# nv-tlabs/LION

Hardware: NVIDIA H100
Metric: shapes/sec (1000-step DDPM, 2048 latent pts, B=32) (higher is better)
Workload: dtype tf32 (fp32 storage/accumulate)

## Files before the change

include/lion_b200.h:

```cpp
#ifndef LION_B200_H
#define LION_B200_H
#include <stddef.h>
#ifdef __cplusplus
extern "C" {
#endif

typedef struct LionCtx LionCtx;
typedef struct LionModel LionModel;

int lion_version(void);
const char* lion_last_error(void);
int lion_ctx_create(int device, LionCtx** out);
int lion_ctx_destroy(LionCtx* ctx);
int lion_ctx_last_launches(LionCtx* ctx);
int lion_ctx_last_conv_group(LionCtx* ctx);
int lion_ctx_last_conv_stage_taps(LionCtx* ctx);
int lion_ctx_set_conv_whole_slabs(LionCtx* ctx, int on);
unsigned lion_ctx_generation(LionCtx* ctx);
int lion_ctx_timeline(LionCtx* ctx, unsigned long long* t_ns, char* names, int max_entries);
size_t lion_ctx_arena_bytes(LionCtx* ctx);
size_t lion_workspace_bytes(LionCtx* ctx);

int lion_avg_voxelize(const float* features, const int* coords, float* out, int* ind, int* cnt,
                      int B, int C, int N, int r, void* stream);
int lion_trilinear_devoxelize(const float* grid, const float* coords, float* out, int* inds, float* wgts,
                              int B, int C, int N, int r, int is_training, void* stream);
int lion_furthest_point_sampling(const float* coords, int* idx, int B, int N, int M, void* stream);
int lion_gather(const float* features, const int* idx, float* out, int B, int C, int N, int M, void* stream);
int lion_ball_query(const float* centers, const float* points, int* out, int B, int N, int M, float radius, int K,
                    void* stream);
int lion_grouping(const float* features, const int* idx, float* out, int B, int C, int N, int M, int U, void* stream);
int lion_three_nn_interpolate(const float* points, const float* centers, const float* centers_features, float* out,
                              int* idx, float* wgt, int B, int C, int N, int M, void* stream);
int lion_voxel_coords(const float* coords, float* norm_coords, int* vox, int B, int N, int r, int normalize, float eps,
                      void* stream);

int lion_avg_voxelize_backward(const float* grad_y , const int* ind , const int* cnt ,
                               float* grad_x , int B, int C, int N, int r, void* stream);
int lion_trilinear_devoxelize_backward(const float* grad_y , const int* inds , const float* wgts ,
                                       float* grad_x , int B, int C, int N, int r, void* stream);
// ... 16 lines not shown
                      int B, int N, void* stream);
#define LION_FWD_CONV_FP16 1
int lion_unet_forward_flags(LionModel* m, const float* x, const float* t, const float* style, const float* clip, float* out,
                            int B, int N, int flags, void* stream);
int lion_unet_cache_style(LionModel* m, const float* style, const float* clip, int B, void* stream);
int lion_style_encoder_forward(LionModel* m, const float* x, float* out, int B, int N, void* stream);
int lion_pvconv_fwd(LionModel* m, const float* features, const float* coords, const float* style, float* out,
                    int B, int N, void* stream);
int lion_sa_module_fwd(LionModel* m, const float* features, const float* coords, const float* style,
                       float* out_features, float* out_coords, int B, int N, void* stream);
int lion_fp_module_fwd(LionModel* m, const float* points_coords, const float* centers_coords,
                       const float* centers_features, const float* points_features, const float* style, float* out,
                       int B, int N, int M, void* stream);
int lion_linear_attention_fwd(LionModel* m, const float* x, float* out, int B, int N, void* stream);
int lion_shared_mlp_fwd(LionModel* m, const float* x, const float* style, float* out, int B, int R, void* stream);
int lion_adagn_fwd(LionModel* m, const float* x, const float* style, float* out, int B, int R, void* stream);
int lion_se3d_fwd(LionCtx* ctx, const float* w1, const float* w2, const float* x, float* out, int B, int C, int V, void* stream);
int lion_swish_fwd(const float* x, float* out, size_t n, void* stream);
int lion_conv3d_gn_fwd(LionModel* m, const float* x, float* out, double* gn_sum, double* gn_sqsum, int B, void* stream);
int lion_conv3d_gn_fwd_flags(LionModel* m, const float* x, float* out, double* gn_sum, double* gn_sqsum, int B, int flags,
                             void* stream);
int lion_pvconv_conv1_probe(LionModel* m, const float* features, const float* coords, int path, float* out,
                            double* gn_sum, double* gn_sqsum, int* path_taken, int B, int N, void* stream);
int lion_sa_mlp_probe(LionModel* m, const float* features, const float* coords, const float* style, int path,
                      float* centers, double* gn_sum, double* gn_sqsum, float* scale, float* shift, float* pool_mm,
                      int* path_taken, int B, int N, void* stream);
int lion_pvconv_probe(LionModel* m, const float* features, const float* coords, const float* style, float* raw1, float* act1,
                      float* raw2, float* rawp, double* sums, float* affine, float* fused, float* out, int* conv2_kernel,
                      int B, int N, void* stream);
int lion_pvconv_probe_flags(LionModel* m, const float* features, const float* coords, const float* style, float* raw1,
                            float* act1, float* raw2, float* rawp, double* sums, float* affine, float* fused, float* out,
                            int* conv2_kernel, int B, int N, int flags, void* stream);
int lion_attention_probe(LionModel* m, const float* x, float* qkv, float* o, float* out, int B, int N, void* stream);
int lion_fp_probe(LionModel* m, const float* points_coords, const float* centers_coords, const float* centers_features,
                  const float* points_features, const float* style, int* nn_idx, float* nn_wgt, float* cat, float* raw,
                  float* act, double* gn_sum, double* gn_sqsum, float* scale, float* shift, int B, int N, int M, void* stream);
int lion_unet_probe(LionModel* m, const float* x, const float* t, const float* style, const float* clip, float* out,
                    void* const* taps, int ntaps, int* style_table, int n_style, int B, int N, void* stream);
int lion_global_prior_forward(LionModel* m, const float* x, const float* t, const float* clip, float* out, int B,
                              void* stream);
int lion_global_prior_probe(LionModel* m, const float* x, const float* t, const float* clip, float* out,
                            void* const* taps, int ntaps, int B, void* stream);
int lion_global_prior_step(LionModel* m, const float* x, const float* t, const float* clip, float* out, int B,
                           void* stream);
size_t lion_global_prior_saved_floats(LionModel* m, int B);
int lion_global_prior_forward_train(LionModel* m, const float* x, const float* t, const float* clip,
// ... 74 lines not shown
```

lion_b200/_lib.py:

```python
import ctypes as C
import os
import threading

import torch

_HERE = os.path.dirname(os.path.abspath(__file__))
LIB_PATH = os.path.join(_HERE, "csrc", "liblion_b200.so")


class LionError(RuntimeError):
    pass


_lib = None
_lock = threading.Lock()
c_f = C.c_void_p


def _proto(lib):
    i, f, d, sz, vp = C.c_int, C.c_float, C.c_double, C.c_size_t, C.c_void_p
    P = lambda *a: list(a)
    sig = {
        "lion_version": ([], i),
        "lion_last_error": ([], C.c_char_p),
        "lion_ctx_create": (P(i, C.POINTER(vp)), i),
        "lion_ctx_destroy": (P(vp), i),
        "lion_ctx_last_launches": (P(vp), i),
        "lion_ctx_last_conv_group": (P(vp), i),
        "lion_ctx_last_conv_stage_taps": (P(vp), i),
        "lion_ctx_set_conv_whole_slabs": (P(vp, i), i),
        "lion_ctx_arena_bytes": (P(vp), sz),
        "lion_ctx_generation": (P(vp), C.c_uint),
        "lion_ctx_timeline": (P(vp, vp, vp, i), i),
        "lion_avg_voxelize": (P(vp, vp, vp, vp, vp, i, i, i, i, vp), i),
        "lion_trilinear_devoxelize": (P(vp, vp, vp, vp, vp, i, i, i, i, i, vp), i),
        "lion_furthest_point_sampling": (P(vp, vp, i, i, i, vp), i),
        "lion_gather": (P(vp, vp, vp, i, i, i, i, vp), i),
        "lion_ball_query": (P(vp, vp, vp, i, i, i, f, i, vp), i),
        "lion_grouping": (P(vp, vp, vp, i, i, i, i, i, vp), i),
        "lion_three_nn_interpolate": (P(vp, vp, vp, vp, vp, vp, i, i, i, i, vp), i),
        "lion_voxel_coords": (P(vp, vp, vp, i, i, i, i, f, vp), i),
        "lion_avg_voxelize_backward": (P(vp, vp, vp, vp, i, i, i, i, vp), i),
        "lion_trilinear_devoxelize_backward": (P(vp, vp, vp, vp, i, i, i, i, vp), i),
        "lion_grouping_backward": (P(vp, vp, vp, i, i, i, i, i, vp), i),
        "lion_three_nn_interpolate_backward": (P(vp, vp, vp, vp, i, i, i, i, vp), i),
        "lion_gather_backward": (P(vp, vp, vp, i, i, i, i, vp), i),
        "lion_model_create": (P(vp, i, C.POINTER(i), i, C.POINTER(vp), i, C.POINTER(vp)), i),
        "lion_model_destroy": (P(vp), i),
        "lion_model_refresh": (P(vp), i),
        "lion_unet_forward": (P(vp, vp, vp, vp, vp, vp, i, i, vp), i),
        "lion_unet_forward_flags": (P(vp, vp, vp, vp, vp, vp, i, i, i, vp), i),
        "lion_unet_cache_style": (P(vp, vp, vp, i, vp), i),
        "lion_style_encoder_forward": (P(vp, vp, vp, i, i, vp), i),
        "lion_pvconv_fwd": (P(vp, vp, vp, vp, vp, i, i, vp), i),
        "lion_sa_module_fwd": (P(vp, vp, vp, vp, vp, vp, i, i, vp), i),
        "lion_fp_module_fwd": (P(vp, vp, vp, vp, vp, vp, vp, i, i, i, vp), i),
        "lion_linear_attention_fwd": (P(vp, vp, vp, i, i, vp), i),
        "lion_shared_mlp_fwd": (P(vp, vp, vp, vp, i, i, vp), i),
        "lion_global_prior_forward": (P(vp, vp, vp, vp, vp, i, vp), i),
        "lion_adagn_fwd": (P(vp, vp, vp, vp, i, i, vp), i),
        "lion_se3d_fwd": (P(vp, vp, vp, vp, vp, i, i, i, vp), i),
        "lion_swish_fwd": (P(vp, vp, sz, vp), i),
        "lion_ddpm_update": (P(vp, vp, vp, vp, vp, vp, f, sz, vp, i, vp), i),
        "lion_ddpm_set_step": (P(vp, vp, i, i, vp), i),
        "lion_ddpm_next_step": (P(vp, vp, i, vp), i),
        "lion_ddpm_fetch_noise": (P(vp, vp, vp, sz, vp), i),
        "lion_conv3d_gn_fwd": (P(vp, vp, vp, vp, vp, i, vp), i),
        "lion_conv3d_gn_fwd_flags": (P(vp, vp, vp, vp, vp, i, i, vp), i),
        "lion_pvconv_conv1_probe": (P(vp, vp, vp, i, vp, vp, vp, C.POINTER(i), i, i, vp), i),
        "lion_sa_mlp_probe": (P(vp, vp, vp, vp, i, vp, vp, vp, vp, vp, vp, C.POINTER(i), i, i, vp), i),
        "lion_pvconv_probe": (P(vp, vp, vp, vp, vp, vp, vp, vp, vp, vp, vp, vp, C.POINTER(i), i, i, vp), i),
        "lion_pvconv_probe_flags": (P(vp, vp, vp, vp, vp, vp, vp, vp, vp, vp, vp, vp, C.POINTER(i), i, i, i, vp), i),
        "lion_attention_probe": (P(vp, vp, vp, vp, vp, i, i, vp), i),
        "lion_fp_probe": (P(vp, vp, vp, vp, vp, vp, vp, vp, vp, vp, vp, vp, vp, vp, vp, i, i, i, vp), i),
        "lion_unet_probe": (P(vp, vp, vp, vp, vp, vp, C.POINTER(vp), i, C.POINTER(i), i, i, i, vp), i),
        "lion_global_prior_step": (P(vp, vp, vp, vp, vp, i, vp), i),
        "lion_global_prior_probe": (P(vp, vp, vp, vp, vp, C.POINTER(vp), i, i, vp), i),
        "lion_global_prior_saved_floats": (P(vp, i), sz),
        "lion_global_prior_forward_train": (P(vp, vp, vp, vp, vp, vp, vp, i, vp), i),
        "lion_global_prior_backward": (P(vp, vp, vp, vp, vp, vp, C.POINTER(vp), i, i, vp), i),
        "lion_global_prior_backward_probe": (P(vp, vp, vp, vp, vp, vp, C.POINTER(vp), i, C.POINTER(vp), i, i, vp), i),
        "lion_workspace_bytes": (P(vp), sz),
        "lion_ddim_update": (P(vp, vp, vp, vp, vp, vp, sz, vp, vp), i),
        "lion_ddim_set_step": (P(vp, vp, vp, i, i, i, vp), i),
        "lion_ddim_next_step": (P(vp, vp, vp, i, i, vp), i),
        "lion_scheduler_step": (P(vp, vp, vp, vp, vp, vp, sz, vp), i),
        "lion_ode_state_bytes": ([], sz),
        "lion_ode_init": (P(vp, vp, vp, sz, d, d, d, d, i, vp), i),
        "lion_ode_stage": (P(vp, vp, vp, vp, sz, i, vp, vp, i, vp), i),
        "lion_ode_rhs": (P(vp, vp, vp, vp, sz, i, d, d, d, vp, vp), i),
        "lion_ode_norms": (P(vp, vp, vp, vp, sz, i, vp, vp), i),
        "lion_ode_control": (P(vp, vp, sz, i, vp), i),
# ... 192 lines not shown
```

lion_b200/csrc/common.cuh:

```cuda
#pragma once
#include <cuda_runtime.h>
#include <cstdint>
#include <cstdio>
#include <cstdarg>
#include <cstring>
#include <string>
#include <vector>
#include <mutex>

namespace lion {

enum : int { LION_OK = 0, LION_ERR_CUDA = -1, LION_ERR_ARG = -2, LION_ERR_OOM = -3, LION_ERR_STATE = -4 };

void set_error(const char* fmt, ...);
const char* get_error();

#define LION_CHECK_CUDA(expr)                                                          \
  do {                                                                                 \
    cudaError_t _e = (expr);                                                           \
    if (_e != cudaSuccess) {                                                           \
      lion::set_error("%s:%d: %s -> %s", __FILE__, __LINE__, #expr, cudaGetErrorString(_e)); \
      return lion::LION_ERR_CUDA;                                                      \
    }                                                                                  \
  } while (0)
// ... 13 lines not shown
  } while (0)

constexpr int LION_MAX_STAMPS = 256;
struct Ctx {
  int device = 0;
  int num_sms = 132;
  int l2_bytes = 50 << 20;
  cudaStream_t stream = nullptr;
  cudaStream_t aux = nullptr;
  char* base = nullptr;
  char* zgrid = nullptr;
  size_t zgrid_cap = 0, zgrid_need = 0;
  size_t cap = 0;
  size_t off = 0;
  size_t peak = 0;
  unsigned generation = 0;
  std::mutex* mu = nullptr;
  bool dry = false;
  int launches = 0;
  int conv_smem_cap = 0;
  int conv_group_blocks = 0;
  int conv_stage_taps = 0;
  bool conv_whole_slabs = false;
  unsigned long long* d_stamps = nullptr;
  int n_stamps = 0;
  char stamp_names[LION_MAX_STAMPS][24];

  void reset() { off = 0; peak = 0; launches = 0; zgrid_need = 0; n_stamps = 0; }
  void* alloc(size_t bytes) {
    size_t a = (off + 255) & ~size_t(255);
    off = a + bytes;
    if (off > peak) peak = off;
    if (dry) return (void*)(uintptr_t)(0x1000 + a);
    return base + a;
  }
  template <typename T> T* alloc_n(size_t n) { return (T*)alloc(n * sizeof(T)); }
  size_t mark() const { return off; }
  void release(size_t m) { off = m; }
};

int ctx_reserve(Ctx* c, size_t bytes);

#define LION_LAUNCH_ON(ctx, stream, kernel, grid, block, smem, ...)                    \
  do {                                                                                 \
    if (!(ctx)->dry) {                                                                 \
      kernel<<<(grid), (block), (smem), (stream)>>>(__VA_ARGS__);                      \
// ... 92 lines not shown
```

lion_b200/csrc/net.cu:

```cuda
#include <algorithm>
#include <deque>
#include <memory>
#include <cstdlib>
#include <cmath>
#include "common.cuh"
#include "packed_kernels.cuh"
#include "model.cuh"
#include "../../include/lion_b200.h"

namespace lion {

static thread_local char g_err[1024] = "";
void set_error(const char* fmt, ...) {
  va_list ap;
  va_start(ap, fmt);
  vsnprintf(g_err, sizeof(g_err), fmt, ap);
  va_end(ap);
}
const char* get_error() { return g_err; }

int ctx_reserve(Ctx* c, size_t bytes) {
  if (bytes <= c->cap) return 0;
  cudaStreamCaptureStatus st = cudaStreamCaptureStatusNone;
  cudaStreamIsCapturing(c->stream, &st);
// ... 454 lines not shown
  if (N > VOXP_MAXN || r > 32) { set_error("voxelisation: N=%d (max %d) or r=%d (max 32) unsupported", N, VOXP_MAXN, r); return LION_ERR_ARG; }
  v.nc = f.c->alloc_n<float4>((size_t)f.B * N);
  v.order = f.c->alloc_n<int>((size_t)f.B * N);
  v.ppos = f.c->alloc_n<int>((size_t)f.B * N);
  v.len = f.c->alloc_n<int>((size_t)f.B * N);
  int P = (r + 2) * (r + 2) * (r + 2);
  v.occ_stride = (P + 63) / 64 + 4;
  v.occ = f.c->alloc_n<unsigned char>((size_t)f.B * v.occ_stride);
  LION_TRY(memset_async(f.c, v.occ, 0, (size_t)f.B * v.occ_stride, s));
  if (sparse_conv1_wanted(N, r)) {
    v.cidx = f.c->alloc_n<int>((size_t)f.B * N);
    v.nocc = f.c->alloc_n<int>((size_t)f.B);
    v.vgrid = f.c->alloc_n<int>((size_t)f.B * P);
    LION_TRY(memset_async(f.c, v.vgrid, 0xff, (size_t)f.B * P * sizeof(int), s));
  }
  LION_LAUNCH_ON(f.c, s, k_vox_prep, f.B, VOXP_THREADS, 0, c4, v.nc, v.order, v.ppos, v.len, v.occ, v.occ_stride, N, r, v.cidx, v.nocc,
                 v.vgrid);
  LION_TRY(check_launch(f.c, "vox_prep"));
  f.vox.push_back(v);
  *out = &f.vox.back();
  return 0;
}

struct Conv1Out { float4* raw = nullptr; double* ssum = nullptr; double* ssq = nullptr; float4* g_in = nullptr; bool sparse = false; };
template <typename F>
static int pvconv_conv1(Fwd& f, const PVConvBlk& p, PF feat, const VoxPrep* vp, int path, Conv1Out& o, F&& after_scatter) {
  const int N = feat.R, r = p.r, rp = r + 2, P = rp * rp * rp, Gin = p.cin / 4, Gout = p.cout / 4;
  ConvGeom geo1 = geom_grid(r);
  geo1.occ = vp->occ; geo1.occ_stride = vp->occ_stride;
  const bool sparse_ok = vp->cidx && ygemm_usable(p.c1y) && feat.G == p.c1y.cin_pad / 4;
  if (path == 2 && !sparse_ok) { set_error("PVConv: the sparse first convolution cannot serve this layer / grid"); return LION_ERR_ARG; }
  if (path == 1 && !conv_tc_usable(p.c1, geo1)) { set_error("PVConv: no tensor-core packing of the first convolution"); return LION_ERR_ARG; }
  const bool sparse1 = path == 0 ? sparse_ok : path == 2;
  o.sparse = sparse1;
  PF xc;
  if (sparse1) {
    xc = alloc_pf(f, Gin, N);
    LION_LAUNCH(f.c, k_scatter_compact, dim3(cdiv(N, 128), Gin, f.B), 128, 0, feat.p, vp->order, vp->cidx, vp->len, vp->nocc, xc.p, Gin, N);
  } else {
    size_t zbytes = sizeof(float4) * ((size_t)f.B * Gin * P + 2 * ((size_t)rp * rp + rp + 8));
    if (zbytes > f.c->zgrid_need) f.c->zgrid_need = zbytes;
    o.g_in = f.c->dry ? (float4*)(uintptr_t)0x1000 : (float4*)f.c->zgrid + ((size_t)rp * rp + rp + 8);
    LION_LAUNCH(f.c, k_scatter, dim3(cdiv(N, 128), Gin, f.B), 128, 0, feat.p, vp->order, vp->ppos, vp->len, o.g_in, Gin, N, P);
  }
  stamp(f.c, f.c->stream, " scatter");
  LION_TRY(after_scatter());
  float4* raw1 = alloc_vg(f, Gout, r);
  o.raw = raw1;
  LION_TRY(poison_vg(f, raw1, Gout, r));
  if (sparse1) {
    const int ld = 27 * p.c1.cout_pad;
    float* y = f.c->alloc_n<float>((size_t)f.B * N * ld);
    LION_TRY(ygemm_run(f.c, p.c1y, xc.p, y, ld, vp->nocc, f.B, N));
    double *s1, *q1;
    LION_TRY(alloc_stats(f, p.c1.cout_pad, &s1, &q1));
    const int nwarp = 4;
    const size_t smem = (size_t)nwarp * (32 * (p.c1.cout_pad + 2) * sizeof(float) + SPG_LIST * sizeof(unsigned));
    static DevOnce attr_once;
    if (attr_once.need()) {
      LION_CHECK_CUDA(cudaFuncSetAttribute(k_sparse_conv_gather<32>, cudaFuncAttributeMaxDynamicSharedMemorySize, 96 * 1024));
      LION_CHECK_CUDA(cudaFuncSetAttribute(k_sparse_conv_gather<64>, cudaFuncAttributeMaxDynamicSharedMemorySize, 96 * 1024));
      LION_CHECK_CUDA(cudaFuncSetAttribute(k_sparse_conv_gather<32>, cudaFuncAttributePreferredSharedMemoryCarveout, cudaSharedmemCarveoutMaxShared));
      LION_CHECK_CUDA(cudaFuncSetAttribute(k_sparse_conv_gather<64>, cudaFuncAttributePreferredSharedMemoryCarveout, cudaSharedmemCarveoutMaxShared));
      LION_CHECK_CUDA(cudaFuncSetAttribute(k_act_grid<false>, cudaFuncAttributePreferredSharedMemoryCarveout, cudaSharedmemCarveoutMaxShared));
      LION_CHECK_CUDA(cudaFuncSetAttribute(k_act_grid<true>, cudaFuncAttributePreferredSharedMemoryCarveout, cudaSharedmemCarveoutMaxShared));
      LION_CHECK_CUDA(cudaFuncSetAttribute(k_scatter_compact, cudaFuncAttributePreferredSharedMemoryCarveout, cudaSharedmemCarveoutMaxShared));
    }
    const dim3 grid(cdiv(r * r * r, 32 * nwarp), f.B);
    if (p.c1.cout_pad == 32)
      LION_LAUNCH(f.c, k_sparse_conv_gather<32>, grid, 32 * nwarp, smem, y, ld, vp->vgrid, p.c1.bias, raw1, s1, q1, p.c1.cout_pad, r, N);
    else
      LION_LAUNCH(f.c, k_sparse_conv_gather<64>, grid, 32 * nwarp, smem, y, ld, vp->vgrid, p.c1.bias, raw1, s1, q1, p.c1.cout_pad, r, N);
    LION_TRY(check_launch(f.c, "sparse conv1"));
    o.ssum = s1; o.ssq = q1;
  } else {
    LION_TRY(alloc_stats(f, p.c1.cout_pad, &o.ssum, &o.ssq));
    LION_TRY(run_conv(f, p.c1, o.g_in, Gin, raw1, Gout, o.ssum, o.ssq, geo1));
  }
  return 0;
}

static int pvconv_fwd(Fwd& f, const PVConvBlk& p, PF feat, const float4* c4, float4* dst, int Gd, int g_off) {
  int N = feat.R, r = p.r, rp = r + 2, P = rp * rp * rp, Gin = p.cin / 4, Gout = p.cout / 4;
  if (feat.G != Gin) { set_error("PVConv: got %d input channels, expected %d", feat.G * 4, p.cin); return LION_ERR_ARG; }
  VoxPrep* vp;
  LION_TRY(get_vox(f, f.c->stream, c4, N, r, &vp));
  size_t mk = f.c->mark();
  ConvGeom geo = geom_grid(r);
  const ConvW& pw = p.point.conv[0];
  PF rawp;
  AffSrc ap;
  PrepJob jp, j1;
  Conv1Out c1;
  LION_TRY(pvconv_conv1(f, p, feat, vp, 0, c1, [&]() -> int {
    rawp = alloc_pf(f, Gout, N);
    return conv_gn_deferred(f, pw, feat.p, feat.G, rawp.p, Gout, geom_rows(N), p.point.gn[0], (double)N, ap, jp);
  }));
  const bool sparse1 = c1.sparse;
  float4 *raw1 = c1.raw, *g_in = c1.g_in;
  AffSrc a1;
  const double V = (double)r * r * r;
  j1 = prep_job(f, p.g1, c1.ssum, c1.ssq, p.c1.cout_pad, V, nullptr, nullptr, a1);
  LION_TRY(run_prep(f, j1, &jp));
  stamp(f.c, f.c->stream, " conv1");
  const bool h2 = f.conv_f16 && p.c2.tc16.w;
  const int Gact = h2 ? Gout / 2 : Gout;
  float4* act1 = alloc_vg(f, Gact, r);
  LION_TRY(poison_vg(f, act1, Gact, r));
  {
    const int nb_act = cdiv(P, 256 * ACT_U);
    const dim3 grid(nb_act + (sparse1 ? 0 : cdiv(N, 256)), Gact, f.B);
    if (h2)
      LION_LAUNCH(f.c, k_act_grid<true>, grid, 256, 0, raw1, act1, a1, Gout, p.cout, rp, P, nb_act, vp->ppos, g_in, Gin, N);
    else
      LION_LAUNCH(f.c, k_act_grid<false>, grid, 256, 0, raw1, act1, a1, Gout, p.cout, rp, P, nb_act, vp->ppos, g_in, Gin, N);
  }
  stamp(f.c, f.c->stream, " act1");
  float4* raw2 = alloc_vg(f, Gout, r);
  LION_TRY(poison_vg(f, raw2, Gout, r));
  AffSrc a2;
  LION_TRY(conv_gn(f, p.c2, act1, Gact, raw2, Gout, geo, p.g2, V, p.se1, p.se2, a2, h2));
  stamp(f.c, f.c->stream, " conv2");
  if (f.pv) {
    PvRecord& R = *f.pv;
    R.raw1 = raw1; R.act1 = act1; R.raw2 = raw2; R.rawp = rawp.p; R.act1_f16 = h2;
    R.a1 = a1; R.ap = ap; R.a2 = a2;
    R.conv2 = !conv_tc_usable(p.c2, geo) ? 0 : f.c->conv_group_blocks ? f.c->conv_group_blocks : 1;
  }
  if (p.has_attn) {
    PF fused = alloc_pf(f, Gout, N);
    LION_LAUNCH(f.c, k_devox_fuse, dim3(cdiv(N, 128), Gout, f.B), 128, 0, raw2, vp->nc, a2.scale, a2.shift, rawp.p, ap,
                fused.p, Gout, p.cout, N, r, P, Gout, 0);
    LION_TRY(check_launch(f.c, "pvconv"));
    if (f.pv) f.pv->fused = fused.p;
    if (Gd != Gout || g_off != 0) {
      PF t = alloc_pf(f, Gout, N);
      LION_TRY(attn_fwd(f, p.attn, fused, t.p, Gout, 0));
      LION_LAUNCH(f.c, k_copy_groups, dim3(cdiv(N, 256), Gout, f.B), 256, 0, t.p, dst, Gout, Gd, g_off, N);
// ... 533 lines not shown
    delete h;
    return LION_ERR_STATE;
  }
  *out = h;
  return 0;
}
extern "C" int lion_ctx_destroy(LionCtx* h) {
  if (!h) return 0;
  if (h->c.base) cudaFree(h->c.base);
  if (h->c.zgrid) cudaFree(h->c.zgrid);
  if (h->c.aux) cudaStreamDestroy(h->c.aux);
  if (h->c.d_stamps) cudaFree(h->c.d_stamps);
  delete h;
  return 0;
}
extern "C" int lion_ctx_last_launches(LionCtx* h) { return h ? h->c.launches : 0; }
extern "C" int lion_ctx_last_conv_group(LionCtx* h) { return h ? h->c.conv_group_blocks : 0; }
extern "C" int lion_ctx_last_conv_stage_taps(LionCtx* h) { return h ? h->c.conv_stage_taps : 0; }
extern "C" int lion_ctx_set_conv_whole_slabs(LionCtx* h, int on) {
  LION_REQUIRE(h, "lion_ctx_set_conv_whole_slabs: null context");
  h->c.conv_whole_slabs = on != 0;
  return 0;
}
extern "C" unsigned lion_ctx_generation(LionCtx* h) { return h ? h->c.generation : 0; }
extern "C" int lion_ctx_timeline(LionCtx* h, unsigned long long* t_ns, char* names, int max_entries) {
  LION_REQUIRE(h && t_ns && names && max_entries >= 0, "lion_ctx_timeline: null argument");
  if (!h->c.d_stamps) { set_error("lion_ctx_timeline: the context was created without LION_TIMELINE=1"); return LION_ERR_STATE; }
  int n = h->c.n_stamps < max_entries ? h->c.n_stamps : max_entries;
  LION_CHECK_CUDA(cudaSetDevice(h->c.device));
  LION_CHECK_CUDA(cudaDeviceSynchronize());
  LION_CHECK_CUDA(cudaMemcpy(t_ns, h->c.d_stamps, (size_t)n * sizeof(unsigned long long), cudaMemcpyDeviceToHost));
  for (int i = 0; i < n; ++i) memcpy(names + (size_t)i * 24, h->c.stamp_names[i], 24);
  return n;
}
extern "C" size_t lion_ctx_arena_bytes(LionCtx* h) { return h ? h->c.cap : 0; }
extern "C" size_t lion_workspace_bytes(LionCtx* h) { return h ? h->c.cap + h->c.zgrid_cap : 0; }

extern "C" int lion_model_create(LionCtx* ctx, int kind, const int* desc, int ndesc, const float* const* params,
                                 int nparams, LionModel** out) {
  LION_REQUIRE(ctx && out && (desc || ndesc == 0) && (params || nparams == 0), "lion_model_create: null argument");
  LION_CHECK_CUDA(cudaSetDevice(ctx->c.device));
  std::unique_ptr<LionModel> h(new LionModel());
  Model* m = &h->m;
  m->ctx = &ctx->c; m->kind = kind;
  m->desc.assign(desc, desc + ndesc);
  m->params.assign(params, params + nparams);
// ... 295 lines not shown
      LION_CHECK_CUDA(cudaMemcpy2DAsync(gn_sum, sizeof(double) * cout, ssum, sizeof(double) * w.cout_pad, sizeof(double) * cout, B,
                                        cudaMemcpyDeviceToDevice, f.c->stream));
      LION_CHECK_CUDA(cudaMemcpy2DAsync(gn_sqsum, sizeof(double) * cout, ssq, sizeof(double) * w.cout_pad, sizeof(double) * cout, B,
                                        cudaMemcpyDeviceToDevice, f.c->stream));
    }
    return check_launch(f.c, "lion_conv3d_gn_fwd");
  });
}

extern "C" int lion_pvconv_conv1_probe(LionModel* h, const float* features, const float* coords, int path, float* out,
                                       double* gn_sum, double* gn_sqsum, int* path_taken, int B, int N, void* stream) {
  LION_REQUIRE(h && h->m.kind == LION_KIND_PVCONV, "lion_pvconv_conv1_probe: not a pvconv model");
  LION_REQUIRE(features && coords && out && gn_sum && gn_sqsum && path >= 0 && path <= 2 && B > 0 && N > 0,
               "lion_pvconv_conv1_probe: bad arguments");
  Model* m = &h->m;
  return two_pass(m, stream, B, [&](Fwd& f) -> int {
    const PVConvBlk& p = m->block->pv;
    const int r = p.r, rp = r + 2, P = rp * rp * rp, Gout = p.cout / 4;
    PF x = to_pf(f, features, m->desc[0], N);
    float4* c4 = to_c4(f, coords, N);
    VoxPrep* vp;
    LION_TRY(get_vox(f, f.c->stream, c4, N, r, &vp));
    Conv1Out c1;
    LION_TRY(pvconv_conv1(f, p, x, vp, path, c1, [] { return 0; }));
    if (!c1.sparse)
      LION_LAUNCH(f.c, k_act_grid<false>, dim3(cdiv(N, 256), Gout, B), 256, 0, c1.raw, nullptr, AffSrc{}, Gout, p.cout, rp, P, 0,
                  vp->ppos, c1.g_in, p.cin / 4, N);
    LION_LAUNCH(f.c, k_vg_to_cm, dim3(cdiv(r * r * r, 256), Gout, B), 256, 0, c1.raw, out, p.cout, Gout, r);
    if (!f.c->dry) {
      LION_CHECK_CUDA(cudaMemcpy2DAsync(gn_sum, sizeof(double) * p.cout, c1.ssum, sizeof(double) * p.c1.cout_pad,
                                        sizeof(double) * p.cout, B, cudaMemcpyDeviceToDevice, f.c->stream));
      LION_CHECK_CUDA(cudaMemcpy2DAsync(gn_sqsum, sizeof(double) * p.cout, c1.ssq, sizeof(double) * p.c1.cout_pad,
                                        sizeof(double) * p.cout, B, cudaMemcpyDeviceToDevice, f.c->stream));
      if (path_taken) *path_taken = c1.sparse ? 2 : 1;
    }
    return check_launch(f.c, "lion_pvconv_conv1_probe");
  });
}

extern "C" int lion_sa_mlp_probe(LionModel* h, const float* features, const float* coords, const float* style, int path,
                                 float* centers, double* gn_sum, double* gn_sqsum, float* scale, float* shift, float* pool_mm,
                                 int* path_taken, int B, int N, void* stream) {
  LION_REQUIRE(h && h->m.kind == LION_KIND_SA, "lion_sa_mlp_probe: not an SA model");
  LION_REQUIRE(features && coords && (style || h->m.desc[4] == 0) && centers && gn_sum && gn_sqsum && scale && shift && pool_mm &&
               path >= 0 && path <= 2 && B > 0 && N > 0, "lion_sa_mlp_probe: bad arguments");
  Model* m = &h->m;
  const SABlk& s = m->block->sa;
  LION_REQUIRE((int)s.mlp.conv.size() <= MLP_REC_MAX, "lion_sa_mlp_probe: more than %d layers", MLP_REC_MAX);
  LION_REQUIRE(path != 2 || sa_fused_usable(s), "lion_sa_mlp_probe: the fused kernels do not serve this module");
  return two_pass(m, stream, B, [&](Fwd& f) -> int {
    MlpRecord rec;
    rec.force = path;
    f.rec = &rec;
    LION_TRY(style_affine_all(f, style ? style : f.c->alloc_n<float>((size_t)B * 4)));
    PF x = to_pf(f, features, s.cfeat, N);
    Level lv{to_c4(f, coords, N), N};
    lv.centers = f.c->alloc_n<float4>((size_t)B * s.m);
    PF o = alloc_pf(f, s.mlp.cout() / 4, s.m);
    LION_TRY(sa_geometry(f, f.c->stream, s, lv, 0));
// ... 314 lines not shown
```

lion_b200/csrc/packed_kernels.cuh:

```cuda
#pragma once
#include <cuda_fp16.h>
#include "common.cuh"
#include "point_core.cuh"
#include "model.cuh"

namespace lion {

__device__ __forceinline__ float4 f4_max(float4 a, float4 b) {
  return make_float4(fmaxf(a.x, b.x), fmaxf(a.y, b.y), fmaxf(a.z, b.z), fmaxf(a.w, b.w));
}
__device__ __forceinline__ float4 f4_scale(float4 a, float s) { return make_float4(a.x * s, a.y * s, a.z * s, a.w * s); }
__device__ __forceinline__ float4 f4_add(float4 a, float4 b) { return make_float4(a.x + b.x, a.y + b.y, a.z + b.z, a.w + b.w); }
__device__ __forceinline__ float4 f4_fma(float4 a, float s, float4 c) {
  return make_float4(fmaf(a.x, s, c.x), fmaf(a.y, s, c.y), fmaf(a.z, s, c.z), fmaf(a.w, s, c.w));
}

__global__ void k_make_coords(const float4* __restrict__ x, float4* __restrict__ c4, int total) {
  int i = blockIdx.x * blockDim.x + threadIdx.x;
  if (i >= total) return;
  float4 v = x[i];
  v.w = 0.0f;
  c4[i] = v;
}

// ... 122 lines not shown
        const unsigned e = list[i0 + k];
        const float* src = yb + (size_t)(e >> 10) * ldy + ((e >> 5) & 31) * C + lane * CPL;
        if (CPL == 2) val[k] = __ldg(reinterpret_cast<const float2*>(src));
        else val[k] = make_float2(__ldg(src), 0.0f);
        jj[k] = (int)(e & 31);
      }
    }
#pragma unroll
    for (int k = 0; k < SPG_BATCH; ++k) {
      if (jj[k] >= 0) {
        float* a = acc + jj[k] * PITCH + lane * CPL;
        a[0] += val[k].x;
        if (CPL == 2) a[1] += val[k].y;
      }
    }
  }
  __syncwarp();
}

template <int C>
__global__ void __launch_bounds__(128)
k_sparse_conv_gather(const float* __restrict__ y, int ldy, const int* __restrict__ vgrid, const float* __restrict__ bias,
                     float4* __restrict__ out, double* __restrict__ ssum, double* __restrict__ ssq, int stat_stride,
                     int r, int Nrows) {
  static_assert(C == 32 || C == 64, "two (or one) channels per lane");
  constexpr int CPL = C / 32;
  constexpr int PITCH = C + 2;
  extern __shared__ float s_acc[];
  __shared__ float s_red[2][4][C];
  const int b = blockIdx.y, lane = threadIdx.x & 31, wid = threadIdx.x >> 5, nw = blockDim.x >> 5;
  const int rp = r + 2, P = rp * rp * rp, V = r * r * r;
  const int q = (blockIdx.x * nw + wid) * 32 + lane;
  const bool live = q < V;
  int p = 0;
  if (live) { int z = q % r, yy = (q / r) % r, x = q / (r * r); p = ((x + 1) * rp + (yy + 1)) * rp + (z + 1); }
  float* acc = s_acc + (size_t)wid * 32 * PITCH;
  const int* vg = vgrid + (size_t)b * P;
  int nb[27];
#pragma unroll
  for (int t = 0; t < 27; ++t) {
    const int off = ((t / 9) - 1) * rp * rp + (((t / 3) % 3) - 1) * rp + ((t % 3) - 1);
    nb[t] = live ? __ldg(vg + p + off) : -1;
  }
  {
    float bv[CPL];
#pragma unroll
    for (int k = 0; k < CPL; ++k) bv[k] = bias ? bias[lane * CPL + k] : 0.0f;
    for (int j = 0; j < 32; ++j)
#pragma unroll
      for (int k = 0; k < CPL; ++k) acc[j * PITCH + lane * CPL + k] = bv[k];
  }
  const float* yb = y + (size_t)b * Nrows * ldy;
  unsigned* list = reinterpret_cast<unsigned*>(s_acc + (size_t)nw * 32 * PITCH) + wid * SPG_LIST;
  int n = 0;
#pragma unroll
  for (int t = 0; t < 27; ++t) {
    const int v = nb[t];
    const unsigned m = __ballot_sync(0xffffffffu, v >= 0);
    if (n + 32 > SPG_LIST) { spg_flush<C>(acc, list, n, yb, ldy, lane); n = 0; }
    if (v >= 0) list[n + __popc(m & ((1u << lane) - 1u))] = ((unsigned)v << 10) | ((unsigned)t << 5) | (unsigned)lane;
    n += __popc(m);
  }
  spg_flush<C>(acc, list, n, yb, ldy, lane);
  if (live) {
#pragma unroll
    for (int g = 0; g < C / 4; ++g) {
      const float* a = acc + lane * PITCH + g * 4;
      out[((size_t)b * (C / 4) + g) * P + p] = make_float4(a[0], a[1], a[2], a[3]);
    }
  }
  float cs[2][CPL], cq[2][CPL];
#pragma unroll
  for (int k = 0; k < CPL; ++k) { cs[0][k] = cs[1][k] = 0.0f; cq[0][k] = cq[1][k] = 0.0f; }
  const int nlive = max(0, min(32, V - ((int)blockIdx.x * nw + wid) * 32));
  for (int j = 0; j < nlive; j += 2) {
#pragma unroll
    for (int h = 0; h < 2; ++h) {
      if (j + h < nlive) {
#pragma unroll
        for (int k = 0; k < CPL; ++k) { const float a = acc[(j + h) * PITCH + lane * CPL + k]; cs[h][k] += a; cq[h][k] = fmaf(a, a, cq[h][k]); }
      }
    }
  }
#pragma unroll
  for (int k = 0; k < CPL; ++k) { s_red[0][wid][lane * CPL + k] = cs[0][k] + cs[1][k]; s_red[1][wid][lane * CPL + k] = cq[0][k] + cq[1][k]; }
  __syncthreads();
  if (threadIdx.x < C) {
    float a = 0.0f, qq = 0.0f;
    for (int w = 0; w < nw; ++w) { a += s_red[0][w][threadIdx.x]; qq += s_red[1][w][threadIdx.x]; }
    atomicAdd(ssum + (size_t)b * stat_stride + threadIdx.x, (double)a);
    atomicAdd(ssq + (size_t)b * stat_stride + threadIdx.x, (double)qq);
  }
}

__global__ void k_scatter(const float4* __restrict__ feat, const int* __restrict__ s_order, const int* __restrict__ s_ppos,
                          const int* __restrict__ s_len, float4* __restrict__ grid, int G, int N, int P) {
  int b = blockIdx.z, g = blockIdx.y;
// ... 249 lines not shown
    double var = gq / n - mean * mean;
    if (var < 0) var = 0;
    const float rstd = (float)(1.0 / sqrt(var + 1e-5));
    const float f = a.fb[(size_t)b * a.fb_stride + c], bb = a.fb[(size_t)b * a.fb_stride + C + c];
    const float ga = a.gamma[c], be = a.beta[c];
    s_aff[threadIdx.x] = rstd * ga * f;
    s_aff[4 + threadIdx.x] = (be - (float)mean * rstd * ga) * f + bb;
  }
  __syncthreads();
  s = make_float4(s_aff[0], s_aff[1], s_aff[2], s_aff[3]);
  t = make_float4(s_aff[4], s_aff[5], s_aff[6], s_aff[7]);
}

constexpr int ACT_U = 4;
__device__ __forceinline__ float4 h8_pack(float4 a, float4 b) {
  union { __half2 h[4]; float4 f; } u;
  u.h[0] = __floats2half2_rn(a.x, a.y); u.h[1] = __floats2half2_rn(a.z, a.w);
  u.h[2] = __floats2half2_rn(b.x, b.y); u.h[3] = __floats2half2_rn(b.z, b.w);
  return u.f;
}

template <bool F16>
__global__ void k_act_grid(const float4* __restrict__ in, float4* __restrict__ out, AffSrc aff, int G, int C, int rp, int P,
                           int nb_act, const int* __restrict__ us_ppos, float4* __restrict__ us_grid, int us_G, int us_N) {
  constexpr int NG = F16 ? 2 : 1;
  int b = blockIdx.z, g = blockIdx.y;
  if ((int)blockIdx.x >= nb_act) {
    int sidx = ((int)blockIdx.x - nb_act) * blockDim.x + threadIdx.x;
    if (sidx >= us_N) return;
    int pp = us_ppos[(size_t)b * us_N + sidx];
    if (pp >= 0)
      for (int gg = g; gg < us_G; gg += gridDim.y) us_grid[((size_t)b * us_G + gg) * P + pp] = make_float4(0.f, 0.f, 0.f, 0.f);
    return;
  }
  float4 s[NG], t[NG];
#pragma unroll
  for (int k = 0; k < NG; ++k) {
    if (k) __syncthreads();
    aff_block_load(aff, b, NG * g + k, C, s[k], t[k]);
  }
  const float4* src = in + ((size_t)b * G + NG * g) * P;
  float4* dst = out + ((size_t)b * (G / NG) + g) * P;
  const int p0 = blockIdx.x * (blockDim.x * ACT_U) + threadIdx.x;
  float4 v[ACT_U][NG];
  bool interior[ACT_U];
  const unsigned rp_m = 0xffffffffu / (unsigned)rp + 1u;
#pragma unroll
  for (int u = 0; u < ACT_U; ++u) {
    int p = p0 + u * blockDim.x;
    const int q = (int)__umulhi((unsigned)p, rp_m), x = (int)__umulhi((unsigned)q, rp_m);
    const int z = p - q * rp, y = q - x * rp;
    interior[u] = p < P && z >= 1 && z <= rp - 2 && y >= 1 && y <= rp - 2 && x >= 1 && x <= rp - 2;
#pragma unroll
    for (int k = 0; k < NG; ++k) {
      v[u][k] = make_float4(0.f, 0.f, 0.f, 0.f);
      if (interior[u]) v[u][k] = __ldcs(src + (size_t)k * P + p);
    }
  }
#pragma unroll
  for (int u = 0; u < ACT_U; ++u) {
    int p = p0 + u * blockDim.x;
    if (p < P) {
      float4 r = make_float4(0.f, 0.f, 0.f, 0.f);
      if (interior[u]) {
        if constexpr (F16) r = h8_pack(f4_swish(f4_affine(v[u][0], s[0], t[0])), f4_swish(f4_affine(v[u][1], s[1], t[1])));
        else r = f4_tf32(f4_swish(f4_affine(v[u][0], s[0], t[0])));
      }
      dst[p] = r;
    }
  }
}

template <int POOL>
__global__ void k_act_rows(const float4* __restrict__ in, float4* __restrict__ out, AffSrc aff, int G, int C, int R_out, int Gd,
                           int g_off, int flags) {
  int b = blockIdx.z, g = blockIdx.y;
  int i = blockIdx.x * blockDim.x + threadIdx.x;
  float4 s, t;
  aff_block_load(aff, b, g, C, s, t);
  if (i >= R_out) return;
  const float4* src = in + ((size_t)b * G + g) * (size_t)R_out * POOL + (size_t)i * POOL;
  float4 r = f4_affine(src[0], s, t);
  if (!(flags & 2)) r = f4_swish(r);
#pragma unroll 4
  for (int k = 1; k < POOL; ++k) r = f4_max(r, f4_swish(f4_affine(src[k], s, t)));
  if (flags & 1) r = f4_tf32(r);
  out[((size_t)b * Gd + g_off + g) * R_out + i] = r;
}

__global__ void k_act_rows_pool32(const float4* __restrict__ in, float4* __restrict__ out, AffSrc aff, int G, int C, int R_out,
                                  int Gd, int g_off) {
// ... 404 lines not shown
```

Before: 3.052.

## Skip raw stores for empty voxel warps in sparse conv1 using occupancy mask

The sparse conv1 gather kernel now writes a per-warp bitmask of output voxels that have at least one occupied neighbour. It skips storing raw outputs for voxels with none, unless whole-output storage is requested. The activation kernel reads this mask and substitutes a precomputed constant, the swish of the affine-transformed bias, for inactive interior voxels instead of loading raw values. This is meant to cut global memory traffic for the sparse voxel grid, at the cost of an extra mask buffer, per-element mask lookups, and a debug flag plus probe to force dense behaviour.

```diff
diff --git a/include/lion_b200.h b/include/lion_b200.h
--- a/include/lion_b200.h
+++ b/include/lion_b200.h
@@ -16,6 +16,7 @@
 int lion_ctx_last_conv_group(LionCtx* ctx);
 int lion_ctx_last_conv_stage_taps(LionCtx* ctx);
 int lion_ctx_set_conv_whole_slabs(LionCtx* ctx, int on);
+int lion_ctx_set_sparse_conv1_dense(LionCtx* ctx, int on);
 unsigned lion_ctx_generation(LionCtx* ctx);
 int lion_ctx_timeline(LionCtx* ctx, unsigned long long* t_ns, char* names, int max_entries);
 size_t lion_ctx_arena_bytes(LionCtx* ctx);
@@ -78,6 +79,8 @@
                              void* stream);
 int lion_pvconv_conv1_probe(LionModel* m, const float* features, const float* coords, int path, float* out,
                             double* gn_sum, double* gn_sqsum, int* path_taken, int B, int N, void* stream);
+int lion_pvconv_conv1_mask_probe(LionModel* m, const float* features, const float* coords, int* vgrid, unsigned* mask, int B,
+                                 int N, void* stream);
 int lion_sa_mlp_probe(LionModel* m, const float* features, const float* coords, const float* style, int path,
                       float* centers, double* gn_sum, double* gn_sqsum, float* scale, float* shift, float* pool_mm,
                       int* path_taken, int B, int N, void* stream);
diff --git a/lion_b200/_lib.py b/lion_b200/_lib.py
--- a/lion_b200/_lib.py
+++ b/lion_b200/_lib.py
@@ -29,6 +29,7 @@
         "lion_ctx_last_conv_group": (P(vp), i),
         "lion_ctx_last_conv_stage_taps": (P(vp), i),
         "lion_ctx_set_conv_whole_slabs": (P(vp, i), i),
+        "lion_ctx_set_sparse_conv1_dense": (P(vp, i), i),
         "lion_ctx_arena_bytes": (P(vp), sz),
         "lion_ctx_generation": (P(vp), C.c_uint),
         "lion_ctx_timeline": (P(vp, vp, vp, i), i),
@@ -68,6 +69,7 @@
         "lion_conv3d_gn_fwd": (P(vp, vp, vp, vp, vp, i, vp), i),
         "lion_conv3d_gn_fwd_flags": (P(vp, vp, vp, vp, vp, i, i, vp), i),
         "lion_pvconv_conv1_probe": (P(vp, vp, vp, i, vp, vp, vp, C.POINTER(i), i, i, vp), i),
+        "lion_pvconv_conv1_mask_probe": (P(vp, vp, vp, vp, vp, i, i, vp), i),
         "lion_sa_mlp_probe": (P(vp, vp, vp, vp, i, vp, vp, vp, vp, vp, vp, C.POINTER(i), i, i, vp), i),
         "lion_pvconv_probe": (P(vp, vp, vp, vp, vp, vp, vp, vp, vp, vp, vp, vp, C.POINTER(i), i, i, vp), i),
         "lion_pvconv_probe_flags": (P(vp, vp, vp, vp, vp, vp, vp, vp, vp, vp, vp, vp, C.POINTER(i), i, i, i, vp), i),
diff --git a/lion_b200/csrc/common.cuh b/lion_b200/csrc/common.cuh
--- a/lion_b200/csrc/common.cuh
+++ b/lion_b200/csrc/common.cuh
@@ -59,6 +59,7 @@
   int conv_group_blocks = 0;
   int conv_stage_taps = 0;
   bool conv_whole_slabs = false;
+  bool sparse_conv1_dense = false;
   unsigned long long* d_stamps = nullptr;
   int n_stamps = 0;
   char stamp_names[LION_MAX_STAMPS][24];
diff --git a/lion_b200/csrc/net.cu b/lion_b200/csrc/net.cu
--- a/lion_b200/csrc/net.cu
+++ b/lion_b200/csrc/net.cu
@@ -500,9 +500,11 @@
   return 0;
 }
 
-struct Conv1Out { float4* raw = nullptr; double* ssum = nullptr; double* ssq = nullptr; float4* g_in = nullptr; bool sparse = false; };
+struct Conv1Out { float4* raw = nullptr; double* ssum = nullptr; double* ssq = nullptr; float4* g_in = nullptr; bool sparse = false;
+                  const unsigned* mask = nullptr; };
 template <typename F>
-static int pvconv_conv1(Fwd& f, const PVConvBlk& p, PF feat, const VoxPrep* vp, int path, Conv1Out& o, F&& after_scatter) {
+static int pvconv_conv1(Fwd& f, const PVConvBlk& p, PF feat, const VoxPrep* vp, int path, bool whole_raw, Conv1Out& o,
+                        F&& after_scatter) {
   const int N = feat.R, r = p.r, rp = r + 2, P = rp * rp * rp, Gin = p.cin / 4, Gout = p.cout / 4;
   ConvGeom geo1 = geom_grid(r);
   geo1.occ = vp->occ; geo1.occ_stride = vp->occ_stride;
@@ -545,12 +547,17 @@
       LION_CHECK_CUDA(cudaFuncSetAttribute(k_scatter_compact, cudaFuncAttributePreferredSharedMemoryCarveout, cudaSharedmemCarveoutMaxShared));
     }
     const dim3 grid(cdiv(r * r * r, 32 * nwarp), f.B);
+    unsigned* mask = f.c->alloc_n<unsigned>((size_t)f.B * cdiv(r * r * r, 32));
+    const bool whole = whole_raw || f.c->sparse_conv1_dense;
     if (p.c1.cout_pad == 32)
-      LION_LAUNCH(f.c, k_sparse_conv_gather<32>, grid, 32 * nwarp, smem, y, ld, vp->vgrid, p.c1.bias, raw1, s1, q1, p.c1.cout_pad, r, N);
+      LION_LAUNCH(f.c, k_sparse_conv_gather<32>, grid, 32 * nwarp, smem, y, ld, vp->vgrid, p.c1.bias, raw1, s1, q1, p.c1.cout_pad, r, N,
+                  mask, whole);
     else
-      LION_LAUNCH(f.c, k_sparse_conv_gather<64>, grid, 32 * nwarp, smem, y, ld, vp->vgrid, p.c1.bias, raw1, s1, q1, p.c1.cout_pad, r, N);
+      LION_LAUNCH(f.c, k_sparse_conv_gather<64>, grid, 32 * nwarp, smem, y, ld, vp->vgrid, p.c1.bias, raw1, s1, q1, p.c1.cout_pad, r, N,
+                  mask, whole);
     LION_TRY(check_launch(f.c, "sparse conv1"));
     o.ssum = s1; o.ssq = q1;
+    o.mask = mask;
   } else {
     LION_TRY(alloc_stats(f, p.c1.cout_pad, &o.ssum, &o.ssq));
     LION_TRY(run_conv(f, p.c1, o.g_in, Gin, raw1, Gout, o.ssum, o.ssq, geo1));
@@ -570,12 +577,13 @@
   AffSrc ap;
   PrepJob jp, j1;
   Conv1Out c1;
-  LION_TRY(pvconv_conv1(f, p, feat, vp, 0, c1, [&]() -> int {
+  LION_TRY(pvconv_conv1(f, p, feat, vp, 0, f.pv != nullptr, c1, [&]() -> int {
     rawp = alloc_pf(f, Gout, N);
     return conv_gn_deferred(f, pw, feat.p, feat.G, rawp.p, Gout, geom_rows(N), p.point.gn[0], (double)N, ap, jp);
   }));
   const bool sparse1 = c1.sparse;
   float4 *raw1 = c1.raw, *g_in = c1.g_in;
+  const unsigned* mask1 = f.c->sparse_conv1_dense ? nullptr : c1.mask;
   AffSrc a1;
   const double V = (double)r * r * r;
   j1 = prep_job(f, p.g1, c1.ssum, c1.ssq, p.c1.cout_pad, V, nullptr, nullptr, a1);
@@ -589,9 +597,11 @@
     const int nb_act = cdiv(P, 256 * ACT_U);
     const dim3 grid(nb_act + (sparse1 ? 0 : cdiv(N, 256)), Gact, f.B);
     if (h2)
-      LION_LAUNCH(f.c, k_act_grid<true>, grid, 256, 0, raw1, act1, a1, Gout, p.cout, rp, P, nb_act, vp->ppos, g_in, Gin, N);
+      LION_LAUNCH(f.c, k_act_grid<true>, grid, 256, 0, raw1, act1, a1, Gout, p.cout, rp, P, nb_act, vp->ppos, g_in, Gin, N, mask1,
+                  p.c1.bias);
     else
-      LION_LAUNCH(f.c, k_act_grid<false>, grid, 256, 0, raw1, act1, a1, Gout, p.cout, rp, P, nb_act, vp->ppos, g_in, Gin, N);
+      LION_LAUNCH(f.c, k_act_grid<false>, grid, 256, 0, raw1, act1, a1, Gout, p.cout, rp, P, nb_act, vp->ppos, g_in, Gin, N, mask1,
+                  p.c1.bias);
   }
   stamp(f.c, f.c->stream, " act1");
   float4* raw2 = alloc_vg(f, Gout, r);
@@ -1171,6 +1181,11 @@
   h->c.conv_whole_slabs = on != 0;
   return 0;
 }
+extern "C" int lion_ctx_set_sparse_conv1_dense(LionCtx* h, int on) {
+  LION_REQUIRE(h, "lion_ctx_set_sparse_conv1_dense: null context");
+  h->c.sparse_conv1_dense = on != 0;
+  return 0;
+}
 extern "C" unsigned lion_ctx_generation(LionCtx* h) { return h ? h->c.generation : 0; }
 extern "C" int lion_ctx_timeline(LionCtx* h, unsigned long long* t_ns, char* names, int max_entries) {
   LION_REQUIRE(h && t_ns && names && max_entries >= 0, "lion_ctx_timeline: null argument");
@@ -1512,10 +1527,10 @@
     VoxPrep* vp;
     LION_TRY(get_vox(f, f.c->stream, c4, N, r, &vp));
     Conv1Out c1;
-    LION_TRY(pvconv_conv1(f, p, x, vp, path, c1, [] { return 0; }));
+    LION_TRY(pvconv_conv1(f, p, x, vp, path, true, c1, [] { return 0; }));
     if (!c1.sparse)
       LION_LAUNCH(f.c, k_act_grid<false>, dim3(cdiv(N, 256), Gout, B), 256, 0, c1.raw, nullptr, AffSrc{}, Gout, p.cout, rp, P, 0,
-                  vp->ppos, c1.g_in, p.cin / 4, N);
+                  vp->ppos, c1.g_in, p.cin / 4, N, nullptr, nullptr);
     LION_LAUNCH(f.c, k_vg_to_cm, dim3(cdiv(r * r * r, 256), Gout, B), 256, 0, c1.raw, out, p.cout, Gout, r);
     if (!f.c->dry) {
       LION_CHECK_CUDA(cudaMemcpy2DAsync(gn_sum, sizeof(double) * p.cout, c1.ssum, sizeof(double) * p.c1.cout_pad,
@@ -1525,6 +1540,26 @@
       if (path_taken) *path_taken = c1.sparse ? 2 : 1;
     }
     return check_launch(f.c, "lion_pvconv_conv1_probe");
+  });
+}
+
+extern "C" int lion_pvconv_conv1_mask_probe(LionModel* h, const float* features, const float* coords, int* vgrid, unsigned* mask,
+                                            int B, int N, void* stream) {
+  LION_REQUIRE(h && h->m.kind == LION_KIND_PVCONV, "lion_pvconv_conv1_mask_probe: not a pvconv model");
+  LION_REQUIRE(features && coords && vgrid && mask && B > 0 && N > 0, "lion_pvconv_conv1_mask_probe: bad arguments");
+  Model* m = &h->m;
+  return two_pass(m, stream, B, [&](Fwd& f) -> int {
+    const PVConvBlk& p = m->block->pv;
+    const int r = p.r, rp = r + 2, P = rp * rp * rp;
+    PF x = to_pf(f, features, m->desc[0], N);
+    float4* c4 = to_c4(f, coords, N);
+    VoxPrep* vp;
+    LION_TRY(get_vox(f, f.c->stream, c4, N, r, &vp));
+    Conv1Out c1;
+    LION_TRY(pvconv_conv1(f, p, x, vp, 2, false, c1, [] { return 0; }));
+    LION_TRY(memcpy_d2d(f.c, vgrid, vp->vgrid, sizeof(int) * (size_t)B * P));
+    LION_TRY(memcpy_d2d(f.c, mask, c1.mask, sizeof(unsigned) * (size_t)B * cdiv(r * r * r, 32)));
+    return check_launch(f.c, "lion_pvconv_conv1_mask_probe");
   });
 }
 
diff --git a/lion_b200/csrc/packed_kernels.cuh b/lion_b200/csrc/packed_kernels.cuh
--- a/lion_b200/csrc/packed_kernels.cuh
+++ b/lion_b200/csrc/packed_kernels.cuh
@@ -168,7 +168,7 @@
 __global__ void __launch_bounds__(128)
 k_sparse_conv_gather(const float* __restrict__ y, int ldy, const int* __restrict__ vgrid, const float* __restrict__ bias,
                      float4* __restrict__ out, double* __restrict__ ssum, double* __restrict__ ssq, int stat_stride,
-                     int r, int Nrows) {
+                     int r, int Nrows, unsigned* __restrict__ mask, bool store_all) {
   static_assert(C == 32 || C == 64, "two (or one) channels per lane");
   constexpr int CPL = C / 32;
   constexpr int PITCH = C + 2;
@@ -199,16 +199,21 @@
   const float* yb = y + (size_t)b * Nrows * ldy;
   unsigned* list = reinterpret_cast<unsigned*>(s_acc + (size_t)nw * 32 * PITCH) + wid * SPG_LIST;
   int n = 0;
+  bool any = false;
 #pragma unroll
   for (int t = 0; t < 27; ++t) {
     const int v = nb[t];
     const unsigned m = __ballot_sync(0xffffffffu, v >= 0);
+    any |= v >= 0;
     if (n + 32 > SPG_LIST) { spg_flush<C>(acc, list, n, yb, ldy, lane); n = 0; }
     if (v >= 0) list[n + __popc(m & ((1u << lane) - 1u))] = ((unsigned)v << 10) | ((unsigned)t << 5) | (unsigned)lane;
     n += __popc(m);
   }
   spg_flush<C>(acc, list, n, yb, ldy, lane);
-  if (live) {
+  const int word = (int)blockIdx.x * nw + wid;
+  const unsigned active = __ballot_sync(0xffffffffu, any);
+  if (lane == 0 && word * 32 < V) mask[(size_t)b * ((V + 31) / 32) + word] = active;
+  if (live && (store_all || any)) {
 #pragma unroll
     for (int g = 0; g < C / 4; ++g) {
       const float* a = acc + lane * PITCH + g * 4;
@@ -218,7 +223,7 @@
   float cs[2][CPL], cq[2][CPL];
 #pragma unroll
   for (int k = 0; k < CPL; ++k) { cs[0][k] = cs[1][k] = 0.0f; cq[0][k] = cq[1][k] = 0.0f; }
-  const int nlive = max(0, min(32, V - ((int)blockIdx.x * nw + wid) * 32));
+  const int nlive = max(0, min(32, V - word * 32));
   for (int j = 0; j < nlive; j += 2) {
 #pragma unroll
     for (int h = 0; h < 2; ++h) {
@@ -514,7 +519,8 @@
 
 template <bool F16>
 __global__ void k_act_grid(const float4* __restrict__ in, float4* __restrict__ out, AffSrc aff, int G, int C, int rp, int P,
-                           int nb_act, const int* __restrict__ us_ppos, float4* __restrict__ us_grid, int us_G, int us_N) {
+                           int nb_act, const int* __restrict__ us_ppos, float4* __restrict__ us_grid, int us_G, int us_N,
+                           const unsigned* __restrict__ mask, const float* __restrict__ bias) {
   constexpr int NG = F16 ? 2 : 1;
   int b = blockIdx.z, g = blockIdx.y;
   if ((int)blockIdx.x >= nb_act) {
@@ -534,8 +540,21 @@
   const float4* src = in + ((size_t)b * G + NG * g) * P;
   float4* dst = out + ((size_t)b * (G / NG) + g) * P;
   const int p0 = blockIdx.x * (blockDim.x * ACT_U) + threadIdx.x;
+  const int r = rp - 2;
+  const unsigned* mb = mask ? mask + (size_t)b * ((r * r * r + 31) / 32) : nullptr;
+  float4 cst = make_float4(0.f, 0.f, 0.f, 0.f);
+  if (mask) {
+    float4 bv[NG];
+#pragma unroll
+    for (int k = 0; k < NG; ++k) {
+      const int c0 = (NG * g + k) * 4;
+      bv[k] = bias ? make_float4(bias[c0], bias[c0 + 1], bias[c0 + 2], bias[c0 + 3]) : make_float4(0.f, 0.f, 0.f, 0.f);
+    }
+    if constexpr (F16) cst = h8_pack(f4_swish(f4_affine(bv[0], s[0], t[0])), f4_swish(f4_affine(bv[1], s[1], t[1])));
+    else cst = f4_tf32(f4_swish(f4_affine(bv[0], s[0], t[0])));
+  }
   float4 v[ACT_U][NG];
-  bool interior[ACT_U];
+  bool interior[ACT_U], active[ACT_U];
   const unsigned rp_m = 0xffffffffu / (unsigned)rp + 1u;
 #pragma unroll
   for (int u = 0; u < ACT_U; ++u) {
@@ -543,22 +562,29 @@
     const int q = (int)__umulhi((unsigned)p, rp_m), x = (int)__umulhi((unsigned)q, rp_m);
     const int z = p - q * rp, y = q - x * rp;
     interior[u] = p < P && z >= 1 && z <= rp - 2 && y >= 1 && y <= rp - 2 && x >= 1 && x <= rp - 2;
+    active[u] = interior[u];
+    if (mb && interior[u]) {
+      const int qi = ((x - 1) * r + (y - 1)) * r + (z - 1);
+      active[u] = (__ldg(mb + (qi >> 5)) >> (qi & 31)) & 1u;
+    }
 #pragma unroll
     for (int k = 0; k < NG; ++k) {
       v[u][k] = make_float4(0.f, 0.f, 0.f, 0.f);
-      if (interior[u]) v[u][k] = __ldcs(src + (size_t)k * P + p);
+      if (active[u]) v[u][k] = __ldcs(src + (size_t)k * P + p);
     }
   }
 #pragma unroll
   for (int u = 0; u < ACT_U; ++u) {
     int p = p0 + u * blockDim.x;
     if (p < P) {
-      float4 r = make_float4(0.f, 0.f, 0.f, 0.f);
-      if (interior[u]) {
-        if constexpr (F16) r = h8_pack(f4_swish(f4_affine(v[u][0], s[0], t[0])), f4_swish(f4_affine(v[u][1], s[1], t[1])));
-        else r = f4_tf32(f4_swish(f4_affine(v[u][0], s[0], t[0])));
+      float4 o = make_float4(0.f, 0.f, 0.f, 0.f);
+      if (active[u]) {
+        if constexpr (F16) o = h8_pack(f4_swish(f4_affine(v[u][0], s[0], t[0])), f4_swish(f4_affine(v[u][1], s[1], t[1])));
+        else o = f4_tf32(f4_swish(f4_affine(v[u][0], s[0], t[0])));
+      } else if (interior[u]) {
+        o = cst;
       }
-      dst[p] = r;
+      dst[p] = o;
     }
   }
 }
```

Result: faster. 3.218, median of 6 (+5.4%).
